# Hengle/AkariRender-1

Measured on AMD Instinct MI355X. Metric: Msamples/sec (whole node), 10M-tri scene 1080p 1024spp, 1/2/4/8 MI355X, higher is better.
Workload: dtype f32; 1 GPU; C3 synthetic triangle soup (SURVEY.md §8d); triangles=10000002, width=1920, height=1080, spp=1025, max_depth=5, tile=64, parallelism=tile-split x1, bvh_leaf=4, builder=sbvh, form=k_path, ordered_fetch=True

## Files before the change

akarirender-1_amd/csrc/kernels.hip:

```cpp
#include "akr_device.h"
#include "akr_math.h"
#include "kernels.h"
#include "leaf_layout.h"

namespace akr {

__device__ __forceinline__ uint32_t fbits(float f) { return __float_as_uint(f); }
__device__ __forceinline__ float bitsf(uint32_t u) { return __uint_as_float(u); }

template <bool TIGHT, bool FAST = false>
__device__ __forceinline__ float box_test(float lox, float hix, float loy, float hiy, float loz, float hiz, V3 o,
                                          V3 invd, float tmin, float tmax) {
    float t0x = (lox - o.x) * invd.x, t1x = (hix - o.x) * invd.x;
    float t0y = (loy - o.y) * invd.y, t1y = (hiy - o.y) * invd.y;
    float t0z = (loz - o.z) * invd.z, t1z = (hiz - o.z) * invd.z;
    float m0, m1, t;
    if (FAST) {
        m0 = fmaxf(fmaxf(fminf(t0x, t1x), fminf(t0y, t1y)), fminf(t0z, t1z));
        m1 = fminf(fminf(fmaxf(t0x, t1x), fmaxf(t0y, t1y)), fmaxf(t0z, t1z));
        t = fmaxf(tmin, m0);
    } else {
        m0 = rmax(rmax(rmin(t0x, t1x), rmin(t0y, t1y)), rmin(t0z, t1z));
        m1 = rmin(rmin(rmax(t0x, t1x), rmax(t0y, t1y)), rmax(t0z, t1z));
        t = rmax(tmin, m0);
// ... 225 lines not shown
            }
        }
    } else {
#pragma unroll
        for (int k = 0; k < 4; k++) {
            if ((rest >> pos[k]) & 1u) {
                const int e = sp + (int)__popc(rest >> (pos[k] + 1u));
                const unsigned long long v = (unsigned long long)ref[k] | ((unsigned long long)__float_as_uint(t[k]) << 32);
                if (e < kStackLds) lds_put(s_stack, e, tid, v);
                else ovf[(size_t)(e - kStackLds) * ovf_threads + gtid] = v;
            }
        }
    }
    sp += (int)__popc(rest);
    const uint32_t first = pm ^ rest;
    uint32_t c = AKR_CHILD_EMPTY;
#pragma unroll
    for (int k = 0; k < 4; k++) c = ((first >> pos[k]) & 1u) ? ref[k] : c;
    cur = c;
    return false;
}

template <bool TIGHT, bool ANY>
__device__ __forceinline__ int visit_wide(const float4 *wn, uint32_t &cur, V3 o, uint32_t dpos, V3 invd, float tmin, float tmax,
                                          float best, lds_u64 *s_stack, glb_u64 *ovf, uint32_t ovf_threads,
                                          uint32_t tid, uint32_t gtid, int &sp) {
    const char *wb = reinterpret_cast<const char *>(wn);
    const uint32_t off = cur << 6;
    const float4 h = *reinterpret_cast<const float4 *>(wb + off);
    const uint4 c = *reinterpret_cast<const uint4 *>(wb + off + 16);
    const uint4 qa = *reinterpret_cast<const uint4 *>(wb + off + 32);
    const uint4 qb = *reinterpret_cast<const uint4 *>(wb + off + 48);
    const uint32_t meta = __float_as_uint(h.w);
    const float sx = __uint_as_float((meta & 0xFFu) << 23);
    const float sy = __uint_as_float(((meta >> 8) & 0xFFu) << 23);
    const float sz = __uint_as_float(((meta >> 16) & 0xFFu) << 23);
    const float lim = ANY ? tmax : best;
    float t[4];
    bool hit[4];
    uint32_t ref[4] = {c.x, c.y, c.z, c.w};
#pragma unroll
    for (int k = 0; k < 4; k++) {
        const float lox = __builtin_fmaf(ubyte(qa.x, k), sx, h.x), hix = __builtin_fmaf(ubyte(qa.y, k), sx, h.x);
        const float loy = __builtin_fmaf(ubyte(qa.z, k), sy, h.y), hiy = __builtin_fmaf(ubyte(qa.w, k), sy, h.y);
        const float loz = __builtin_fmaf(ubyte(qb.x, k), sz, h.z), hiz = __builtin_fmaf(ubyte(qb.y, k), sz, h.z);
        t[k] = box_test<TIGHT, true>(lox, hix, loy, hiy, loz, hiz, o, invd, tmin, tmax);
        hit[k] = ref[k] != AKR_CHILD_EMPTY && !(t[k] < 0.0f || t[k] > lim);
    }
    const int tested = (c.x != AKR_CHILD_EMPTY) + (c.y != AKR_CHILD_EMPTY) + (c.z != AKR_CHILD_EMPTY) +
                       (c.w != AKR_CHILD_EMPTY);
    wide_order_push<ANY>(qb.z, qb.w, dpos, t, hit, ref, cur, lim, s_stack, ovf, ovf_threads, tid, gtid, sp);
    return tested;
}

struct WideNode {
    float4 h;
    uint4 c, qa, qb;
};
__device__ __forceinline__ WideNode wide_load(const float4 *wn, uint32_t cur) {
    const char *wb = reinterpret_cast<const char *>(wn);
    const uint32_t off = cur << 6;
    WideNode nd;
    nd.h = *reinterpret_cast<const float4 *>(wb + off);
    nd.c = *reinterpret_cast<const uint4 *>(wb + off + 16);
    nd.qa = *reinterpret_cast<const uint4 *>(wb + off + 32);
    nd.qb = *reinterpret_cast<const uint4 *>(wb + off + 48);
    return nd;
}

__device__ __forceinline__ float max3_raw(float a, float b, float c, float d) {
    float m, r;
    asm("v_max_f32 %0, %1, %2" : "=v"(m) : "v"(c), "v"(d));
    asm("v_max3_f32 %0, %1, %2, %3" : "=v"(r) : "v"(a), "v"(b), "v"(m));
    return r;
}
__device__ __forceinline__ float min3_raw(float a, float b, float c, float d) {
    float m, r;
    asm("v_min_f32 %0, %1, %2" : "=v"(m) : "v"(c), "v"(d));
    asm("v_min3_f32 %0, %1, %2, %3" : "=v"(r) : "v"(a), "v"(b), "v"(m));
    return r;
}

constexpr bool kTrimMinMax = true, kTrimPush = true;
template <bool ANY, bool NOPOP = false, bool FIT = false, bool TRIM = false>
__device__ __forceinline__ int visit_wide_lean_node(const WideNode &nd, uint32_t &cur, V3 o, uint32_t dpos, V3 invd,
                                                    float tmin, float tmaxp, float best, lds_u64 *s_stack, glb_u64 *ovf,
                                                    uint32_t ovf_threads, uint32_t tid, uint32_t gtid, int &sp,
                                                    bool *need_pop = nullptr, lds_u64 *dead = nullptr,
                                                    uint32_t *push_info = nullptr, uint32_t *entered = nullptr) {
    const float4 h = nd.h;
    const uint4 c = nd.c, qa = nd.qa, qb = nd.qb;
    const uint32_t meta = __float_as_uint(h.w);
    constexpr float kRel = 0x1p-21f;
    constexpr float kAbs = 0x1p-120f;
    const float scx = __uint_as_float((meta & 0xFFu) << 23) * invd.x;
    const float scy = __uint_as_float(((meta >> 8) & 0xFFu) << 23) * invd.y;
    const float scz = __uint_as_float(((meta >> 16) & 0xFFu) << 23) * invd.z;
    const float oqx = (h.x - o.x) * invd.x, oqy = (h.y - o.y) * invd.y, oqz = (h.z - o.z) * invd.z;
    const float ex = __builtin_fmaf(__builtin_fmaf(255.0f, fabsf(scx), fabsf(oqx)), kRel, kAbs);
    const float ey = __builtin_fmaf(__builtin_fmaf(255.0f, fabsf(scy), fabsf(oqy)), kRel, kAbs);
    const float ez = __builtin_fmaf(__builtin_fmaf(255.0f, fabsf(scz), fabsf(oqz)), kRel, kAbs);
    const float nox = oqx - ex, noy = oqy - ey, noz = oqz - ez;
    const float fox = oqx + ex, foy = oqy + ey, foz = oqz + ez;
    const bool px = invd.x > 0.0f, py = invd.y > 0.0f, pz = invd.z > 0.0f;
    const uint32_t qnx = px ? qa.x : qa.y, qfx = px ? qa.y : qa.x;
    const uint32_t qny = py ? qa.z : qa.w, qfy = py ? qa.w : qa.z;
    const uint32_t qnz = pz ? qb.x : qb.y, qfz = pz ? qb.y : qb.x;
    const float lim = ANY || TRIM ? tmaxp : fminf(best, tmaxp);
    float t[4];
    bool hit[4];
    uint32_t ref[4] = {c.x, c.y, c.z, c.w};
#pragma unroll
    for (int k = 0; k < 4; k++) {
        const float nx = __builtin_fmaf(ubyte(qnx, k), scx, nox), fx = __builtin_fmaf(ubyte(qfx, k), scx, fox);
        const float ny = __builtin_fmaf(ubyte(qny, k), scy, noy), fy = __builtin_fmaf(ubyte(qfy, k), scy, foy);
        const float nz = __builtin_fmaf(ubyte(qnz, k), scz, noz), fz = __builtin_fmaf(ubyte(qfz, k), scz, foz);
        constexpr bool RAW = TRIM && kTrimMinMax;
        const float tk = RAW ? max3_raw(nx, ny, nz, tmin) : fmaxf(fmaxf(nx, ny), fmaxf(nz, tmin));
        const float m1 = RAW ? min3_raw(fx, fy, fz, lim) : fminf(fminf(fx, fy), fminf(fz, lim));
        t[k] = tk;
        hit[k] = ref[k] != AKR_CHILD_EMPTY && tk <= m1;
    }
    const int tested = (c.x != AKR_CHILD_EMPTY) + (c.y != AKR_CHILD_EMPTY) + (c.z != AKR_CHILD_EMPTY) +
                       (c.w != AKR_CHILD_EMPTY);
    const bool np = wide_order_push<ANY, NOPOP, FIT, TRIM && kTrimPush>(qb.z, qb.w, dpos, t, hit, ref, cur, ANY ? tmaxp : best, s_stack, ovf,
                                                     ovf_threads, tid, gtid, sp, dead, push_info, entered);
    if (NOPOP) *need_pop = np;
    return tested;
}

template <bool ANY>
__device__ __forceinline__ int visit_wide_lean(const float4 *wn, uint32_t &cur, V3 o, uint32_t dpos, V3 invd, float tmin,
                                               float tmaxp, float best, lds_u64 *s_stack, glb_u64 *ovf,
                                               uint32_t ovf_threads, uint32_t tid, uint32_t gtid, int &sp) {
    const WideNode nd = wide_load(wn, cur);
    return visit_wide_lean_node<ANY>(nd, cur, o, dpos, invd, tmin, tmaxp, best, s_stack, ovf, ovf_threads, tid, gtid, sp);
}

__device__ __forceinline__ float float_below(float x) {
    const uint32_t b = __float_as_uint(x);
    if (x > 0.0f) return __uint_as_float(b - 1u);
    if (x == 0.0f) return -0x1p-149f;
    return __uint_as_float(b + 1u);
}

__device__ __forceinline__ bool lean_ok(V3 o, V3 invd, float tmin, float tmax) {
    const float mo = fmaxf(fmaxf(fabsf(o.x), fabsf(o.y)), fabsf(o.z));
    const float mi = fmaxf(fmaxf(fabsf(invd.x), fabsf(invd.y)), fabsf(invd.z));
    return fast_box_ok(o, invd, tmin, tmax) && tmin >= 0.0f && tmax > -INFINITY && mo <= 0x1p60f && mi <= 0x1p64f;
}

template <int MODE>
__device__ __forceinline__ void emit_result(const TraceArgs &a, uint32_t idx, float best, float bu, float bv,
                                            uint32_t bgid, bool occluded) {
    constexpr bool ANY = MODE != TRACE_CLOSEST;
    if (MODE == TRACE_SHADOW) {
        if (!occluded) {
            const float4 c = a.shadow_color[idx];
            const uint32_t slot = fbits(c.w);
            float4 l = a.L[slot];
            l.x += c.x;
            l.y += c.y;
            l.z += c.z;
            a.L[slot] = l;
        }
    } else if (a.abi_hits) {
// ... 1066 lines not shown
    unsigned long long tv_issue = 0, tv_wait = 0, tv_comp = 0, tl_issue = 0, tl_wait = 0, tl_comp = 0;
    unsigned long long lphases = 0, lholders = 0;
    unsigned long long pop_iters = 0, pop_rounds = 0, push_iters = 0, push_slow = 0, push_would_fit = 0;
    unsigned long long pop_lane_rounds = 0, pop_lanes = 0;
    bool deep_now = false;
    uint32_t *lines = nullptr;
    uint32_t span[3] = {0, 0, 0};
    const float4 *leaf_base = nullptr;
};

__device__ __forceinline__ void mark_lines(uint32_t *map, uint32_t lo, uint32_t hi, const void *region, const void *p,
                                           uint32_t bytes) {
    const uint64_t r0 = (uint64_t)region >> 7, a = (uint64_t)p;
    if (a < (uint64_t)region) return;
    for (uint64_t l = (a >> 7) - r0; l <= ((a + bytes - 1) >> 7) - r0; l++) {
        const uint64_t b = lo + l;
        if (b < hi) atomicOr(map + (b >> 5), 1u << (b & 31u));
    }
}

template <bool COUNT, bool OVF>
__device__ __forceinline__ void pop_bounded(bool need_pop, PathRay &r, const lds_u64 *s_stack, const glb_u64 *ovf,
                                            uint32_t ovf_threads, uint32_t tid, uint32_t gtid, uint32_t keep,
                                            uint32_t max_rounds, PathCount &c) {
    bool unserved = need_pop;
    uint32_t got = AKR_CHILD_POP;
    int sp = r.sp;
    uint32_t rounds = 0;
    while (true) {
        const bool has = unserved & (sp > 0);
        unsigned long long e;
        if constexpr (!OVF) {
            e = lds_get(s_stack, min(max(sp, 1), kStackLds) - 1, tid);
        } else {
            e = 0;
            if (has) {
                if (sp - 1 < kStackLds) e = lds_get(s_stack, sp - 1, tid);
                else e = ovf[(size_t)(sp - 1 - kStackLds) * ovf_threads + gtid];
            }
        }
        const bool ok = !(__uint_as_float((uint32_t)(e >> 32)) > r.best);
        const uint32_t got_entry = ok ? (uint32_t)e : got, got_none = unserved ? AKR_CHILD_EMPTY : got;
        got = has ? got_entry : got_none;
        sp -= has ? 1 : 0;
        if (COUNT) c.pop_lane_rounds += has ? 1 : 0;
        unserved = has & !ok;
        rounds++;
        if ((uint32_t)__popcll(__ballot(unserved)) < keep || rounds >= max_rounds) break;
    }
    if (COUNT) c.pop_rounds += rounds;
    r.sp = sp;
    if (need_pop) r.cur = got;
}

__device__ __forceinline__ unsigned long long mask_of(bool cmp) { return __builtin_amdgcn_ballot_w64(cmp); }
__device__ __forceinline__ bool in_mask(unsigned long long m) { return __builtin_amdgcn_inverse_ballot_w64(m); }
__device__ __forceinline__ uint32_t lane_count(unsigned long long m) {
    uint32_t n = (uint32_t)__popcll(m);
    asm("" : "+s"(n));
    return n;
}

__device__ __forceinline__ void pop_bounded_lds(unsigned long long need, PathRay &r, const lds_u64 *s_stack, uint32_t tid,
                                                uint32_t keep, uint32_t max_rounds) {
    unsigned long long unserved = need;
    uint32_t got = AKR_CHILD_POP;
    int sp = r.sp;
    uint32_t rounds = 0;
    while (true) {
        const unsigned long long has = unserved & mask_of(sp > 0);
        const unsigned long long e = lds_get(s_stack, min(max(sp, 1), kStackLds) - 1, tid);
        const unsigned long long cull = mask_of(__uint_as_float((uint32_t)(e >> 32)) > r.best);
        got = in_mask(unserved & ~has) ? AKR_CHILD_EMPTY : got;
        got = in_mask(has & ~cull) ? (uint32_t)e : got;
        sp -= in_mask(has) ? 1 : 0;
        unserved = has & cull;
        rounds++;
        if (lane_count(unserved) < (rounds < max_rounds ? keep : 65u)) break;
    }
    r.sp = sp;
    r.cur = in_mask(need) ? got : r.cur;
}

template <int EXIT>
__device__ __forceinline__ void path_traverse_masks(unsigned long long bm, PathRay &r, const float4 *wn, lds_u64 *s_stack,
                                                    glb_u64 *ovf, uint32_t ovf_threads, uint32_t tid, uint32_t gtid,
                                                    uint32_t pop_keep, uint32_t pop_rounds, lds_u64 *dead) {
    static_assert(EXIT >= 0 && EXIT < 64, "the exit test below counts a searching lane without a holder as 65");
    PathCount none;
    const float lim = fminf(r.best, r.tmaxp);
    while (true) {
        uint32_t pm = 1u;
        [[maybe_unused]] bool np;
        if (in_mask(bm & mask_of(is_internal(r.cur)))) {
            const WideNode nd = wide_load(wn, r.cur);
            visit_wide_lean_node<false, true, true, true>(nd, r.cur, r.o, r.dpos, r.invd, r.tmin, lim, r.best, s_stack,
                                                          ovf, ovf_threads, tid, gtid, r.sp, &np, dead, nullptr, &pm);
        }
        asm("" : "+v"(pm));
        unsigned long long need = mask_of(pm == 0);
        const unsigned long long no_leaf = mask_of(r.leaf == AKR_CHILD_EMPTY);
        const unsigned long long post = bm & ~need & no_leaf & mask_of(is_leaf(r.cur));
        r.leaf = in_mask(post) ? r.cur : r.leaf;
        need |= post | (bm & mask_of(r.cur == AKR_CHILD_POP));
        if (need != 0) {
            if (__builtin_expect((need & mask_of(r.sp > kStackLds)) == 0, 1))
                pop_bounded_lds(need, r, s_stack, tid, pop_keep, pop_rounds);
            else
                pop_bounded<false, true>(in_mask(need), r, s_stack, ovf, ovf_threads, tid, gtid, pop_keep, pop_rounds, none);
        }
        const unsigned long long free_now = bm & no_leaf & ~post;
        const unsigned long long searching = free_now & mask_of(r.cur != AKR_CHILD_EMPTY);
        const unsigned long long holders = bm & ~free_now;
        const uint32_t n = lane_count(searching);
        uint32_t left = holders != 0 ? n : n * 65u;
        asm("" : "+s"(left));
        if (left <= (uint32_t)EXIT) break;
    }
}

template <bool COUNT, int EXIT = kWhileExit, bool BOUND = false>
__device__ __forceinline__ void path_traverse(bool busy, int kind, PathRay &r, const float4 *wn, lds_u64 *s_stack,
                                              glb_u64 *ovf, uint32_t ovf_threads, uint32_t tid, uint32_t gtid,
                                              PathCount &c, uint32_t pop_keep = 1, uint32_t pop_rounds = 255,
                                              lds_u64 *dead = nullptr) {
    constexpr bool FIT = BOUND;
    while (true) {
        [[maybe_unused]] unsigned long long tc = 0;
        bool need_pop = false;
        if constexpr (COUNT) {
            c.strav++;
            c.sleaf += busy ? 1 : 0;
            c.iters++;
            const bool vis = busy && is_internal(r.cur);
            const unsigned long long ta = wall_clock64();
            const WideNode nd = wide_load(wn, vis ? r.cur : 0u);
            const unsigned long long tb = wall_clock64();
            asm volatile("s_waitcnt vmcnt(0)" ::: "memory");
            tc = wall_clock64();
            c.tv_issue += tb - ta;
            c.tv_wait += tc - tb;
            uint32_t pinfo = 0;
            if (vis) {
                const uint32_t node = r.cur;
                const int nt = visit_wide_lean_node<false, true, FIT>(nd, r.cur, r.o, r.dpos, r.invd, r.tmin, r.tmaxp,
                                                                      r.best, s_stack, ovf, ovf_threads, tid, gtid, r.sp,
                                                                      &need_pop, dead, &pinfo);
                c.box[kind] += nt;
                c.visit[kind]++;
                c.deep_now = c.deep_now || r.sp > kStackLds;
                if (c.lines)
                    mark_lines(c.lines, 0u, c.span[1], wn, reinterpret_cast<const char *>(wn) + ((size_t)node << 6), 64u);
            }
            if (__ballot(pinfo & 1u) != 0) {
                c.push_iters++;
                if (__ballot(pinfo & 2u) != 0) {
                    c.push_slow++;
                    c.push_would_fit += __ballot(pinfo & 4u) == 0 ? 1 : 0;
                }
            }
        } else if (busy && is_internal(r.cur)) {
            const WideNode nd = wide_load(wn, r.cur);
            visit_wide_lean_node<false, true, FIT>(nd, r.cur, r.o, r.dpos, r.invd, r.tmin, r.tmaxp, r.best, s_stack, ovf,
                                                   ovf_threads, tid, gtid, r.sp, &need_pop, dead);
        }
        if (busy && !need_pop && r.leaf == AKR_CHILD_EMPTY && is_leaf(r.cur)) {
            r.leaf = r.cur;
            need_pop = true;
        }
        if constexpr (BOUND) {
            need_pop = need_pop || (busy && r.cur == AKR_CHILD_POP);
            const unsigned long long want = __ballot(need_pop);
            if (want != 0) {
                if (COUNT) {
                    c.pop_iters++;
                    c.pop_lanes += need_pop ? 1 : 0;
                }
                if (__builtin_expect(__ballot(need_pop && r.sp > kStackLds) == 0, 1))
                    pop_bounded<COUNT, false>(need_pop, r, s_stack, ovf, ovf_threads, tid, gtid, pop_keep, pop_rounds, c);
                else
                    pop_bounded<COUNT, true>(need_pop, r, s_stack, ovf, ovf_threads, tid, gtid, pop_keep, pop_rounds, c);
            }
        } else {
            if (need_pop) r.cur = stack_pop(s_stack, ovf, ovf_threads, tid, gtid, r.sp, r.best);
        }
        const unsigned long long searching = __ballot(busy && r.leaf == AKR_CHILD_EMPTY && r.cur != AKR_CHILD_EMPTY);
        if constexpr (COUNT) {
            const bool stop = (uint32_t)__popcll(searching) <= (uint32_t)EXIT &&
                              (searching == 0 || __ballot(busy && r.leaf != AKR_CHILD_EMPTY) != 0);
            c.tv_comp += wall_clock64() - tc;
            if (stop) break;
        } else if ((uint32_t)__popcll(searching) <= (uint32_t)EXIT &&
                   (searching == 0 || __ballot(busy && r.leaf != AKR_CHILD_EMPTY) != 0)) {
            break;
        }
    }
}

template <bool COUNT>
// ... 9 lines not shown
    const uint32_t cnt = in ? fbits(l1.w) : 0u;
    const float4 *tp = lr + 2;
    for (uint32_t k = 0; k < cnt; k++) {
        if (COUNT && lane_prefix(__ballot(1)) == 0) c.stri += 64;
        const float4 ta = k == 0 ? pa0 : (k == 1 ? pa1 : tp[3 * k + 0]);
        const float4 tb = k == 0 ? pb0 : (k == 1 ? pb1 : tp[3 * k + 1]);
        const float4 tc = k == 0 ? pc0 : (k == 1 ? pc1 : tp[3 * k + 2]);
        if (COUNT) {
            c.tri[kind]++;
            if (c.lines && k >= 2) mark_lines(c.lines, c.span[1], c.span[2], c.leaf_base, tp + 3 * k, 48u);
        }
        float t, u, v;
        if (mt(r.o, r.d, r.tmin, r.tmax, ta, tb, tc, r.best, t, u, v)) {
            r.best = t;
            r.bu = u;
            r.bv = v;
            r.bgid = fbits(ta.w);
            if (kind) {
                hit_any = true;
                break;
            }
        }
    }
    r.leaf = AKR_CHILD_EMPTY;
    return hit_any;
}

template <bool COUNT>
__device__ __forceinline__ bool path_leaf(bool busy, int kind, PathRay &r, const float4 *wide_leaves, PathCount &c) {
    if constexpr (!COUNT) {
        bool hit_any = false;
        if (busy && r.leaf != AKR_CHILD_EMPTY) {
            const float4 *lr = wide_leaves + (r.leaf & kLeafOffsetMask);
            const float4 l0 = lr[0], l1 = lr[1];
            const float4 pa0 = lr[2], pb0 = lr[3], pc0 = lr[4];
            const float4 pa1 = lr[5], pb1 = lr[6], pc1 = lr[7];
            issue_together(pa0, pb0, pc0, pa1, pb1, pc1);
            const float tl = box_test<true, true>(l0.x, l0.w, l0.y, l1.x, l0.z, l1.y, r.o, r.invd, r.tmin, r.tmax);
            const bool in = !(tl < 0.0f || tl > r.best);
            const uint32_t cnt = in ? fbits(l1.w) : 0u;
            const float4 *tp = lr + 2;
            for (uint32_t k = 0; k < cnt; k++) {
                const float4 ta = k == 0 ? pa0 : (k == 1 ? pa1 : tp[3 * k + 0]);
                const float4 tb = k == 0 ? pb0 : (k == 1 ? pb1 : tp[3 * k + 1]);
                const float4 tc = k == 0 ? pc0 : (k == 1 ? pc1 : tp[3 * k + 2]);
                float t, u, v;
                if (mt(r.o, r.d, r.tmin, r.tmax, ta, tb, tc, r.best, t, u, v)) {
                    r.best = t;
                    r.bu = u;
                    r.bv = v;
                    r.bgid = fbits(ta.w);
                    if (kind) {
                        hit_any = true;
                        break;
                    }
                }
            }
            r.leaf = AKR_CHILD_EMPTY;
        }
        return hit_any;
    } else {
        bool hit_any = false;
        const unsigned long long ta = wall_clock64();
        const bool in_leaf = busy && r.leaf != AKR_CHILD_EMPTY;
        const uint32_t holders = (uint32_t)__popcll(__ballot(in_leaf));
        c.lphases += holders ? 1u : 0u;
        c.lholders += holders;
        const float4 *lr = wide_leaves + (in_leaf ? (r.leaf & kLeafOffsetMask) : 0u);
        const float4 l0 = lr[0], l1 = lr[1], pa0 = lr[2], pb0 = lr[3], pc0 = lr[4], pa1 = lr[5], pb1 = lr[6],
                     pc1 = lr[7];
        const unsigned long long tb = wall_clock64();
        asm volatile("s_waitcnt vmcnt(0)" ::: "memory");
        const unsigned long long tc = wall_clock64();
        if (in_leaf && c.lines) mark_lines(c.lines, c.span[1], c.span[2], wide_leaves, lr, 128u);
        if (in_leaf) hit_any = leaf_tests<true>(kind, r, lr, l0, l1, pa0, pb0, pc0, pa1, pb1, pc1, c);
        c.tl_issue += tb - ta;
        c.tl_wait += tc - tb;
        c.tl_comp += wall_clock64() - tc;
        return hit_any;
    }
}

__device__ __forceinline__ unsigned long long path_leaf_masks(unsigned long long bm, unsigned long long am, PathRay &r,
                                                              const float4 *wide_leaves) {
    const unsigned long long hold = bm & mask_of(r.leaf != AKR_CHILD_EMPTY);
    const unsigned long long one = hold & mask_of((r.leaf & kLeafOne) != 0);
    unsigned long long hm = 0;
    const bool several = hold != one;
    if (__builtin_expect(one != 0 && !several, 1)) {
        const float4 *lr = wide_leaves + (in_mask(one) ? (r.leaf & kLeafOffsetMask) : 0u);
        const float4 l0 = lr[0], l1 = lr[1];
        const float4 a = lr[2], b = lr[3], c = lr[4];
        const float tl = box_test<true, true>(l0.x, l0.w, l0.y, l1.x, l0.z, l1.y, r.o, r.invd, r.tmin, r.tmax);
        const unsigned long long out = mask_of(tl < 0.0f) | mask_of(tl > r.best);
        const V3 v0{a.x, a.y, a.z}, e1{b.x, b.y, b.z}, e2{c.x, c.y, c.z};
        const V3 h = cross(r.d, e2);
        const float det = dot(e1, h);
        const unsigned long long flat = mask_of(det > -1e-6f) & mask_of(det < 1e-6f);
        const float f = 1.0f / det;
        const V3 s = sub(r.o, v0);
        const float u = f * dot(s, h);
        const unsigned long long out_u = mask_of(u < 0.0f) | mask_of(u > 1.0f);
        const V3 q = cross(s, e1);
        const float v = f * dot(r.d, q);
        const unsigned long long out_v = mask_of(v < 0.0f) | mask_of(u + v > 1.0f);
        const float t = f * dot(e2, q);
        const unsigned long long near = mask_of(t > r.tmin) & mask_of(t < r.tmax) & mask_of(t < r.best);
        const unsigned long long hit = one & near & ~(out | flat | out_u | out_v);
        const bool won = in_mask(hit);
        r.best = won ? t : r.best;
        r.bu = won ? u : r.bu;
        r.bv = won ? v : r.bv;
        r.bgid = won ? fbits(a.w) : r.bgid;
        r.leaf = in_mask(one) ? AKR_CHILD_EMPTY : r.leaf;
        hm = hit & am;
    }
    if (__builtin_expect(several, 0)) {
        PathCount none{};
        hm |= mask_of(path_leaf<false>(in_mask(bm), in_mask(am) ? 1 : 0, r, wide_leaves, none));
    }
    return hm;
}

template <bool COUNT>
__device__ __forceinline__ bool path_begin(const TraceArgs &a, bool occl, float4 ra, float4 rb, PathRay &r,
                                           lds_u64 *s_stack, glb_u64 *ovf, uint32_t tid, uint32_t gtid, PathCount &c) {
    r.o = V3{ra.x, ra.y, ra.z};
    r.d = V3{rb.x, rb.y, rb.z};
    r.tmin = ra.w;
    r.tmax = rb.w;
    r.invd = V3{1.0f / r.d.x, 1.0f / r.d.y, 1.0f / r.d.z};
    r.dpos = (r.d.x > 0.0f ? 1u : 0u) | (r.d.y > 0.0f ? 2u : 0u) | (r.d.z > 0.0f ? 4u : 0u);
    if (occl && a.any_far_first) r.dpos ^= 7u;
    r.tmaxp = float_below(r.tmax);
    if (COUNT) c.rays[occl]++;
    if (!lean_ok(r.o, r.invd, r.tmin, r.tmax)) {
        bool hit;
        if (occl)
            trace_exact_core<true, true>(a, r.o, r.d, r.invd, r.tmin, r.tmax, s_stack, ovf, tid, gtid, r.best, r.bu,
                                         r.bv, r.bgid, hit);
        else
            trace_exact_core<false, true>(a, r.o, r.d, r.invd, r.tmin, r.tmax, s_stack, ovf, tid, gtid, r.best, r.bu,
                                          r.bv, r.bgid, hit);
        return false;
    }
    r.best = occl ? r.tmax : kInf;
    r.bu = r.bv = 0.0f;
    r.bgid = kNoHit;
    r.sp = 0;
    r.leaf = AKR_CHILD_EMPTY;
    if (COUNT) {
        c.box[occl]++;
        c.deep_now = false;
    }
    const float4 *nodesf = reinterpret_cast<const float4 *>(a.nodes);
    const float4 r0 = nodesf[0], r2 = nodesf[2];
    const float tr = box_test<true, true>(r0.x, r0.y, r0.z, r0.w, r2.x, r2.y, r.o, r.invd, r.tmin, r.tmax);
    r.cur = (a.wide_root == AKR_CHILD_EMPTY || tr < 0.0f || tr > r.best) ? AKR_CHILD_EMPTY : a.wide_root;
    return true;
}

__device__ __forceinline__ void path_park(uint32_t (*s_park)[kTraceBlock], uint32_t tid, const PathRay &r);
__device__ __forceinline__ void path_unpark(uint32_t (*s_park)[kTraceBlock], uint32_t tid, PathRay &r, bool far_first,
                                            bool occl);

struct PixelFetch {
    uint32_t shard, s_lo, s_hi;
    int shards_left;
    bool drained;
    uint32_t stride = 0;
};
__device__ __forceinline__ uint32_t gcd_u32(uint32_t x, uint32_t y) {
    while (y) {
        const uint32_t t = x % y;
        x = y;
        y = t;
    }
    return x;
}
__device__ __forceinline__ void fetch_pixels(PixelFetch &f, uint32_t n, uint32_t *work, uint32_t mode,
                                             const uint32_t *order, uint32_t prio, bool &need, bool &done,
                                             uint32_t &pix) {
    while (true) {
        const unsigned long long want = __ballot(need && !done);
        if (want == 0) break;
        if (f.drained) {
            if (need) done = true;
            break;
        }
        const uint32_t nw = (uint32_t)__popcll(want);
        const int leader = __ffsll((long long)want) - 1;
        uint32_t base = 0;
        if ((int)__lane_id() == leader) base = atomicAdd(work + f.shard * kWorkStride, nw);
        base = __builtin_amdgcn_readfirstlane(__shfl(base, leader));
        const uint32_t len = f.s_hi - f.s_lo;
        if (prio && base < len) {
            if ((uint64_t)base * 256u < (uint64_t)len * prio) __builtin_amdgcn_s_setprio(2);
            else __builtin_amdgcn_s_setprio(0);
        }
        if (need && !done) {
            const uint32_t my = base + lane_prefix(want);
            if (base < len && my < len) {
// ... 61 lines not shown
        atomicAdd(&q.pop_iters, c.pop_iters);
        atomicAdd(&q.pop_rounds, c.pop_rounds);
        atomicAdd(&q.push_iters, c.push_iters);
        atomicAdd(&q.push_slow, c.push_slow);
        atomicAdd(&q.push_would_fit, c.push_would_fit);
    }
    const unsigned long long plr = wave_sum(c.pop_lane_rounds), pln = wave_sum(c.pop_lanes);
    if (__lane_id() == 0 && pa.prof) {
        atomicAdd(&pa.prof->pop_lane_rounds, plr);
        atomicAdd(&pa.prof->pop_lanes, pln);
    }
    const int slot_of[2] = {TRACE_CLOSEST, TRACE_SHADOW};
    for (int m = 0; m < 2; m++) {
        const unsigned long long rr = wave_sum(c.rays[m]), b = wave_sum(c.box[m]), t = wave_sum(c.tri[m]),
                                 v = wave_sum(c.visit[m]), dp = wave_sum(c.deep[m]), lf = wave_sum(c.leaf[m]);
        if (__lane_id() == 0) {
            TraceCounters &tc = a.counters[slot_of[m]];
            atomicAdd(&tc.rays, rr);
            atomicAdd(&tc.box, b);
            atomicAdd(&tc.tri, t);
            atomicAdd(&tc.visits, v);
            atomicAdd(&tc.deep, dp);
            atomicAdd(&tc.leaves, lf);
        }
    }
    const unsigned long long st = wave_sum(c.strav), sl = wave_sum(c.sleaf), sr = wave_sum(c.stri);
    if (__lane_id() == 0) {
        atomicAdd(&a.counters[TRACE_CLOSEST].slots_trav, st);
        atomicAdd(&a.counters[TRACE_CLOSEST].slots_leaf, sl);
        atomicAdd(&a.counters[TRACE_CLOSEST].slots_tri, sr);
    }
}

template <bool COUNT>
__device__ __forceinline__ uint32_t probe_flags(const PathArgs &pa) {
    if (!COUNT) return AKR_PROBE_SEED;
    uint32_t f = AKR_PROBE_SEED | AKR_PROBE_RAYS;
    if (pa.probe_clock) f |= 4u | (uint32_t)((wall_clock64() >> 4) << 8);
    return f;
}

constexpr int kParkSlots = 8;

template <bool COUNT, bool TAB, bool ONE, bool SIMPLE, bool ENV = false>
__device__ __forceinline__ void path_plain(const PathArgs &pa, const EnvDev *env = nullptr) {
    if (pa.gate && *pa.gate != pa.gate_want) return;
    const TraceArgs &a = pa.t;
    __shared__ unsigned long long s_stack_mem[kStackLdsU64];
    __shared__ uint32_t s_park[kParkSlots][kTraceBlock];
    __shared__ uint4 s_tab[TAB ? kTabBytes / 16 : 1];
    lds_u64 *s_stack = (lds_u64 *)s_stack_mem;
    glb_u64 *stack_ovf = (glb_u64 *)a.stack_ovf;
    const uint32_t tid = threadIdx.x;
    const uint32_t gtid = blockIdx.x * kTraceBlock + tid;
    const uint32_t n = pa.n_pix;
    const int nb = pa.max_depth == 0 ? 1 : pa.max_depth;
    const bool ff = a.any_far_first != 0;
    const auto tab = PathTab<TAB>::make(pa.sc, s_tab);
    static_assert(kParkSlots >= 1 && kTraceBlock % 64 == 0, "the push's scratch words lie in a wave's park row 0");
    lds_u64 *dead = (lds_u64 *)&s_park[0][0] + (tid >> 1);
    PathCount c;
    if (COUNT) {
        c.lines = pa.lines;
        c.span[1] = pa.lines_span[1];
        c.span[2] = pa.lines_span[2];
        c.leaf_base = a.wide_leaves;
    }
    PixelFetch f{blockIdx.x % kWorkShards, 0, 0, (int)kWorkShards, n == 0};
    f.s_lo = shard_begin(n, f.shard);
    f.s_hi = shard_begin(n, f.shard + 1);

    uint32_t pix = 0, left = 0, seed = 0, pxr = 0;
    int depth = 0;
    V3 beta{1.0f, 1.0f, 1.0f}, Lr{0.0f, 0.0f, 0.0f}, scol{0.0f, 0.0f, 0.0f};
    float4 film = {0.0f, 0.0f, 0.0f, 0.0f};
    float4 pe0 = {}, pe1 = {};
    enum : uint32_t { F_BUSY = 1u, F_DONE = 2u, F_FIN = 4u, F_NEED = 8u, F_ANY = 16u, F_PEND = 32u };
    uint32_t fl = F_NEED;
    uint32_t pc_closest = 0, pc_shadow = 0;
    PathRay r{};
    r.best = kInf;
    r.bgid = kNoHit;
    r.cur = r.leaf = AKR_CHILD_EMPTY;
    unsigned long long p_outer = 0, p_procs = 0, p_tp = 0, p_tt = 0, p_tl = 0, p_lanes = 0, p_t0 = 0, p_t = 0, p_tsh = 0;
    unsigned long long p_tpark = 0, p_tnext = 0, p_tbegin = 0, p_tload = 0;
    if (COUNT) p_t0 = wall_clock64();

    while (true) {
        const unsigned long long waiting = mask_of((fl & (F_BUSY | F_DONE)) == 0);
        const uint32_t nwait = (uint32_t)__popcll(waiting);
        const uint32_t nbusy = (uint32_t)__popcll(mask_of((fl & F_BUSY) != 0));
        if (nwait == 0 && nbusy == 0) break;
        if (COUNT) {
            p_outer++;
            p_t = wall_clock64();
        }
        if (nwait > 0 && 64u * nwait >= pa.min_wait * (nwait + nbusy)) {
            if (COUNT) {
                p_procs++;
                p_lanes += nwait;
            }
            bool busy = (fl & F_BUSY) != 0, done = (fl & F_DONE) != 0, fin = (fl & F_FIN) != 0;
            bool need_pixel = (fl & F_NEED) != 0, any = (fl & F_ANY) != 0, pend = (fl & F_PEND) != 0;
            path_park(s_park, tid, r);
            __builtin_amdgcn_fence(__ATOMIC_RELEASE, "workgroup");
            asm volatile("" ::: "memory");
            bool fresh = false, next_any = false, sample_end = false, start = false;
            float4 ra = {}, rb = {};
            unsigned long long p_ts = 0;
            unsigned long long tl_phase = 0;
            if (COUNT) {
                p_ts = wall_clock64();
                p_tpark += p_ts - p_t;
            }
            if (!busy && !done && fin) {
                fin = false;
                const uint32_t hgid = r.bgid;
                [[maybe_unused]] const EnvDev *envp = env;
                if constexpr (ENV) {
                    unsigned long long eb = (unsigned long long)env;
                    asm volatile("" : "+s"(eb));
                    envp = (const EnvDev *)(const AKR_GLOBAL EnvDev *)eb;
                }
                if (any) {
                    if (hgid == kNoHit) {
                        Lr.x += scol.x;
                        Lr.y += scol.y;
                        Lr.z += scol.z;
                    }
                    if (pend) {
                        ra = pe0;
                        rb = pe1;
                        fresh = true;
                        pend = false;
                    } else {
                        sample_end = true;
                    }
                } else if (hgid == kNoHit) {
                    if constexpr (ENV) {
                        if (depth == 0) {
                            const V3 d{bitsf(s_park[3][tid]), bitsf(s_park[4][tid]), bitsf(s_park[5][tid])};
                            int ti, tj;
                            float len;
                            env_encode(envp->n, env_to_map(*envp, d), ti, tj, len);
                            const V3 e = mul(beta, env_lookup(*envp, ti, tj));
                            Lr.x += e.x;
                            Lr.y += e.y;
                            Lr.z += e.z;
                        }
                    }
                    sample_end = true;
                } else {
                    const V3 wo{-bitsf(s_park[3][tid]), -bitsf(s_park[4][tid]), -bitsf(s_park[5][tid])};
                    Bounce bo;
                    if (COUNT && pa.lines)
                        mark_lines(pa.lines, pa.lines_span[2], pa.lines_span[3], pa.sc.tri, pa.sc.tri + hgid,
                                   (uint32_t)sizeof(ShadeTri));
                    shade_hit_path<SIMPLE, ENV>(pa.sc, tab, hgid, r.bu, r.bv, wo, beta, seed, depth,
                                                pa.max_depth, depth == nb - 1, bo, COUNT ? &tl_phase : nullptr, envp);
                    if (bo.emit) {
                        Lr.x += bo.e.x;
                        Lr.y += bo.e.y;
                        Lr.z += bo.e.z;
                    }
                    if (bo.ext) {
                        beta = bo.nb;
                        depth++;
                    }
                    if (bo.sh) {
                        ra = bo.s0;
                        rb = bo.s1;
                        scol = bo.col;
                        next_any = true;
                        fresh = true;
                        pend = bo.ext;
                        pe0 = bo.e0;
                        pe1 = bo.e1;
                    } else if (bo.ext) {
                        ra = bo.e0;
                        rb = bo.e1;
                        fresh = true;
                    } else {
                        sample_end = true;
                    }
                }
            }
            if (COUNT) {
                const unsigned long long t = wall_clock64();
                p_tsh += t - p_ts;
                p_ts = t;
                p_tload += wave_max(tl_phase);
            }
            if (sample_end) {
                splat_one(film, make_float4(Lr.x, Lr.y, Lr.z, 0.0f), pa.ray_clamp);
                if (--left == 0) {
                    pa.film[pix] = film;
                    if (pa.state_out) pa.state_out[pix] = seed;
                    if (pa.probe)
                        pa.probe[pix] = make_uint4(seed, COUNT ? pc_closest : 0u, COUNT ? pc_shadow : 0u,
                                                   probe_flags<COUNT>(pa));
                    need_pixel = true;
                } else {
                    start = true;
                }
            }
            const bool asked = need_pixel && !done;
            fetch_pixels(f, n, pa.work, pa.order ? pa.order_mode : FETCH_LINEAR, pa.order, pa.prio, need_pixel, done, pix);
            if (asked && !need_pixel) {
                const uint32_t px = pa.pixel[pix];
                pxr = px;
                left = pa.spp;
                if (pa.state_in) {
                    seed = pa.state_in[pix];
                    film = pa.film[pix];
                } else {
                    seed = (uint32_t)((int)(px & 0xFFFFu) + (int)(px >> 16) * pa.cam.width);
                    film = make_float4(0.0f, 0.0f, 0.0f, 0.0f);
                }
                start = true;
                if (COUNT) pc_closest = pc_shadow = 0;
            }
            if (start) {
                Lr = V3{0.0f, 0.0f, 0.0f};
                beta = V3{1.0f, 1.0f, 1.0f};
                depth = 0;
                const uint32_t px = pxr;
                camera_ray(pa.cam, (int)(px & 0xFFFFu), (int)(px >> 16), seed, ra, rb);
                fresh = true;
            }
            asm volatile("" ::: "memory");
            if (COUNT) {
                const unsigned long long t = wall_clock64();
                p_tnext += t - p_ts;
                p_ts = t;
            }
            path_unpark(s_park, tid, r, ff, any);
            if (fresh) {
                any = next_any;
                if (COUNT) {
                    pc_closest += any ? 0u : 1u;
                    pc_shadow += any ? 1u : 0u;
                }
                busy = path_begin<COUNT>(a, any, ra, rb, r, s_stack, stack_ovf, tid, gtid, c);
                fin = !busy;
            }
            fl = (busy ? F_BUSY : 0u) | (done ? F_DONE : 0u) | (fin ? F_FIN : 0u) | (need_pixel ? F_NEED : 0u) |
                 (any ? F_ANY : 0u) | (pend ? F_PEND : 0u);
            asm("" : "+v"(fl));
            if (COUNT) p_tbegin += wall_clock64() - p_ts;
        }
        if (COUNT) {
            const unsigned long long t = wall_clock64();
            p_tp += t - p_t;
            p_t = t;
        }
        const unsigned long long bm = mask_of((fl & F_BUSY) != 0);
        if (bm == 0) continue;
        const bool busy = in_mask(bm);
        [[maybe_unused]] const int kd = (fl & F_ANY) != 0 ? 1 : 0;
        if constexpr (COUNT)
            path_traverse<COUNT, kWhileExitPath, true>(busy, kd, r, a.wide_nodes, s_stack, stack_ovf, a.ovf_threads, tid,
                                                       gtid, c, pa.pop_keep, pa.pop_rounds, dead);
        else
            path_traverse_masks<kWhileExitPath>(bm, r, a.wide_nodes, s_stack, stack_ovf, a.ovf_threads, tid, gtid,
                                                pa.pop_keep, pa.pop_rounds, dead);
        if (COUNT) {
            const unsigned long long t = wall_clock64();
            p_tt += t - p_t;
            p_t = t;
        }
        bool ended;
        if constexpr (COUNT || !ONE) {
            const bool hit_any = path_leaf<COUNT>(busy, kd, r, a.wide_leaves, c);
            ended = busy && (hit_any || r.cur == AKR_CHILD_EMPTY);
        } else {
            const unsigned long long hm = path_leaf_masks(bm, mask_of((fl & F_ANY) != 0), r, a.wide_leaves);
            ended = in_mask(bm & (hm | mask_of(r.cur == AKR_CHILD_EMPTY)));
        }
        fl = ended ? (fl ^ (F_BUSY | F_FIN)) : fl;
        if (COUNT && ended) c.deep[kd] += c.deep_now ? 1 : 0;
        if (COUNT) p_tl += wall_clock64() - p_t;
    }
    if (COUNT) {
        path_count_flush(pa, c, p_outer, p_procs, p_tp, p_tt, p_tl, p_t0, p_lanes, p_tsh);
        if (__lane_id() == 0 && pa.prof) {
            atomicAdd(&pa.prof->tp_park, p_tpark);
            atomicAdd(&pa.prof->tp_next, p_tnext);
            atomicAdd(&pa.prof->tp_begin, p_tbegin);
            atomicAdd(&pa.prof->tp_load, p_tload);
        }
    }
}

template <bool COUNT, bool TAB>
__global__ __launch_bounds__(kTraceBlock) __attribute__((amdgpu_waves_per_eu(AKR_PATH_WAVES))) void k_path(PathArgs pa) {
    path_plain<COUNT, TAB, true, !COUNT>(pa);
}
template <bool TAB, bool SIMPLE>
__global__ __launch_bounds__(kTraceBlock) __attribute__((amdgpu_waves_per_eu(AKR_PATH_WAVES))) void k_path_general(PathArgs pa) {
    path_plain<false, TAB, false, SIMPLE>(pa);
}
template <bool COUNT, bool TAB>
__global__ __launch_bounds__(kTraceBlock) __attribute__((amdgpu_waves_per_eu(AKR_PATH_WAVES))) void k_path_env(PathEnvArgs ea) {
    path_plain<COUNT, TAB, true, !COUNT, true>(ea.p, (const EnvDev *)ea.env);
}
template <bool TAB, bool SIMPLE>
__global__ __launch_bounds__(kTraceBlock) __attribute__((amdgpu_waves_per_eu(AKR_PATH_WAVES))) void k_path_env_general(PathEnvArgs ea) {
    path_plain<false, TAB, false, SIMPLE, true>(ea.p, (const EnvDev *)ea.env);
}

__device__ __forceinline__ void path_park(uint32_t (*s_park)[kTraceBlock], uint32_t tid, const PathRay &r) {
    const float pv[8] = {r.o.x, r.o.y, r.o.z, r.d.x, r.d.y, r.d.z, r.tmin, r.tmax};
#pragma unroll
    for (int k = 0; k < 8; k++) s_park[k][tid] = fbits(pv[k]);
}
__device__ __forceinline__ void path_unpark(uint32_t (*s_park)[kTraceBlock], uint32_t tid, PathRay &r, bool far_first,
                                            bool occl) {
    r.o = V3{bitsf(s_park[0][tid]), bitsf(s_park[1][tid]), bitsf(s_park[2][tid])};
    r.d = V3{bitsf(s_park[3][tid]), bitsf(s_park[4][tid]), bitsf(s_park[5][tid])};
    r.tmin = bitsf(s_park[6][tid]);
    r.tmax = bitsf(s_park[7][tid]);
    r.invd = V3{1.0f / r.d.x, 1.0f / r.d.y, 1.0f / r.d.z};
    r.dpos = (r.d.x > 0.0f ? 1u : 0u) | (r.d.y > 0.0f ? 2u : 0u) | (r.d.z > 0.0f ? 4u : 0u);
    if (occl && far_first) r.dpos ^= 7u;
    r.tmaxp = float_below(r.tmax);
    r.leaf = AKR_CHILD_EMPTY;
}

__device__ __forceinline__ int nth_set_bit(unsigned long long m, uint32_t r) {
    int base = 0;
#pragma unroll
    for (int s = 32; s > 0; s >>= 1) {
        const unsigned long long low = m & ((1ull << s) - 1ull);
        const uint32_t c = (uint32_t)__popcll(low);
        if (r >= c) {
            r -= c;
            m >>= s;
            base += s;
        } else {
            m = low;
        }
    }
    return base;
}

constexpr uint32_t kDeferSlots = 8;
enum : uint32_t { RAY_NONE = 0, RAY_OWN = 1, RAY_OWN_SHADOW = 2, RAY_FOREIGN = 3 };

struct DeferState {
    uint32_t w = 0;
    static constexpr uint32_t KIND = 0, RP = 2, LAST = 3, OPEN = 4, NSH = 6, DEPTH = 14, FTAG = 18, PEND = 30, RUN = 31;
    __device__ __forceinline__ uint32_t get(uint32_t off, uint32_t bits) const { return (w >> off) & ((1u << bits) - 1u); }
    __device__ __forceinline__ void set(uint32_t off, uint32_t bits, uint32_t v) {
        const uint32_t m = ((1u << bits) - 1u) << off;
        w = (w & ~m) | ((v << off) & m);
    }
    __device__ __forceinline__ uint32_t kind() const { return get(KIND, 2); }
    __device__ __forceinline__ uint32_t rp() const { return get(RP, 1); }
    __device__ __forceinline__ uint32_t last() const { return get(LAST, 1); }
// ... 1298 lines not shown
```

Baseline: 621.1 Msamples/s.

## Prefetch next wide BVH node across loop iterations and trim leaf loads

Issues the load of the next internal wide node at the end of each traversal iteration, after leaf processing and after ray begin, and carries it in registers so the next visit starts with data already in flight. Inline asm barriers keep the node registers live and grouped with the leaf loads so the memory latency overlaps the leaf test. Leaf fetches shrink to float2/float3 loads where only some components are used. The node limit switches to float_below(tmax). This adds around 16 VGPRs of live state per lane, which can lower occupancy, and the change spans several call sites whose consistency must hold.

```diff
diff --git a/akarirender-1_amd/csrc/kernels.hip b/akarirender-1_amd/csrc/kernels.hip
--- a/akarirender-1_amd/csrc/kernels.hip
+++ b/akarirender-1_amd/csrc/kernels.hip
@@ -331,6 +331,26 @@
 }
 
 constexpr bool kTrimMinMax = true, kTrimPush = true;
+constexpr bool kNodeAhead = true;
+__device__ __forceinline__ void node_together(const WideNode &nd) {
+    asm volatile("" ::"v"(nd.h.x), "v"(nd.h.y), "v"(nd.h.z), "v"(nd.h.w), "v"(nd.c.x), "v"(nd.c.y), "v"(nd.c.z),
+                 "v"(nd.c.w), "v"(nd.qa.x), "v"(nd.qa.y), "v"(nd.qa.z), "v"(nd.qa.w), "v"(nd.qb.x), "v"(nd.qb.y),
+                 "v"(nd.qb.z), "v"(nd.qb.w));
+}
+__device__ __forceinline__ void node_forget(WideNode &nd) {
+    asm volatile("" : "=v"(nd.h.x), "=v"(nd.h.y), "=v"(nd.h.z), "=v"(nd.h.w), "=v"(nd.c.x), "=v"(nd.c.y), "=v"(nd.c.z),
+                 "=v"(nd.c.w), "=v"(nd.qa.x), "=v"(nd.qa.y), "=v"(nd.qa.z), "=v"(nd.qa.w), "=v"(nd.qb.x),
+                 "=v"(nd.qb.y), "=v"(nd.qb.z), "=v"(nd.qb.w));
+}
+__device__ __forceinline__ void node_here(WideNode &nd) {
+    asm volatile("" : "+v"(nd.h.x), "+v"(nd.h.y), "+v"(nd.h.z), "+v"(nd.h.w), "+v"(nd.c.x), "+v"(nd.c.z), "+v"(nd.qa.x),
+                 "+v"(nd.qa.y), "+v"(nd.qa.z), "+v"(nd.qa.w), "+v"(nd.qb.x), "+v"(nd.qb.y), "+v"(nd.qb.z),
+                 "+v"(nd.qb.w));
+    uint32_t c1, c3;
+    asm volatile("v_mov_b32 %0, %2\n\tv_mov_b32 %1, %3" : "=&v"(c1), "=&v"(c3) : "v"(nd.c.y), "v"(nd.c.w));
+    nd.c.y = c1;
+    nd.c.w = c3;
+}
 template <bool ANY, bool NOPOP = false, bool FIT = false, bool TRIM = false>
 __device__ __forceinline__ int visit_wide_lean_node(const WideNode &nd, uint32_t &cur, V3 o, uint32_t dpos, V3 invd,
                                                     float tmin, float tmaxp, float best, lds_u64 *s_stack, glb_u64 *ovf,
@@ -1563,19 +1583,24 @@
     r.cur = in_mask(need) ? got : r.cur;
 }
 
-template <int EXIT>
+__device__ __forceinline__ void node_ahead(unsigned long long vm, WideNode &nd, const float4 *wn, uint32_t cur) {
+    node_forget(nd);
+    if (in_mask(vm)) nd = wide_load(wn, cur);
+}
+template <int EXIT, bool AHEAD>
 __device__ __forceinline__ void path_traverse_masks(unsigned long long bm, PathRay &r, const float4 *wn, lds_u64 *s_stack,
                                                     glb_u64 *ovf, uint32_t ovf_threads, uint32_t tid, uint32_t gtid,
-                                                    uint32_t pop_keep, uint32_t pop_rounds, lds_u64 *dead) {
+                                                    uint32_t pop_keep, uint32_t pop_rounds, lds_u64 *dead, WideNode &nd) {
     static_assert(EXIT >= 0 && EXIT < 64, "the exit test below counts a searching lane without a holder as 65");
     PathCount none;
-    const float lim = fminf(r.best, r.tmaxp);
+    const float lim = fminf(r.best, AHEAD ? float_below(r.tmax) : r.tmaxp);
     while (true) {
         uint32_t pm = 1u;
         [[maybe_unused]] bool np;
         if (in_mask(bm & mask_of(is_internal(r.cur)))) {
-            const WideNode nd = wide_load(wn, r.cur);
-            visit_wide_lean_node<false, true, true, true>(nd, r.cur, r.o, r.dpos, r.invd, r.tmin, lim, r.best, s_stack,
+            WideNode now = AHEAD ? nd : wide_load(wn, r.cur);
+            if constexpr (AHEAD) node_here(now);
+            visit_wide_lean_node<false, true, true, true>(now, r.cur, r.o, r.dpos, r.invd, r.tmin, lim, r.best, s_stack,
                                                           ovf, ovf_threads, tid, gtid, r.sp, &np, dead, nullptr, &pm);
         }
         asm("" : "+v"(pm));
@@ -1596,6 +1621,7 @@
         const uint32_t n = lane_count(searching);
         uint32_t left = holders != 0 ? n : n * 65u;
         asm("" : "+s"(left));
+        if constexpr (AHEAD) node_ahead(bm & mask_of(is_internal(r.cur)), nd, wn, r.cur);
         if (left <= (uint32_t)EXIT) break;
     }
 }
@@ -1771,15 +1797,25 @@
 }
 
 __device__ __forceinline__ unsigned long long path_leaf_masks(unsigned long long bm, unsigned long long am, PathRay &r,
-                                                              const float4 *wide_leaves) {
+                                                              const float4 *wide_leaves, WideNode &nd, const float4 *wn) {
     const unsigned long long hold = bm & mask_of(r.leaf != AKR_CHILD_EMPTY);
     const unsigned long long one = hold & mask_of((r.leaf & kLeafOne) != 0);
     unsigned long long hm = 0;
     const bool several = hold != one;
     if (__builtin_expect(one != 0 && !several, 1)) {
         const float4 *lr = wide_leaves + (in_mask(one) ? (r.leaf & kLeafOffsetMask) : 0u);
-        const float4 l0 = lr[0], l1 = lr[1];
-        const float4 a = lr[2], b = lr[3], c = lr[4];
+        const float4 l0 = lr[0];
+        const float2 l1h = *reinterpret_cast<const float2 *>(lr + 1);
+        const float4 l1 = kNodeAhead ? make_float4(l1h.x, l1h.y, 0.0f, 0.0f) : lr[1];
+        const float4 a = lr[2];
+        const float3 b3 = *reinterpret_cast<const float3 *>(lr + 3), c3 = *reinterpret_cast<const float3 *>(lr + 4);
+        const float4 b = kNodeAhead ? make_float4(b3.x, b3.y, b3.z, 0.0f) : lr[3];
+        const float4 c = kNodeAhead ? make_float4(c3.x, c3.y, c3.z, 0.0f) : lr[4];
+        if constexpr (kNodeAhead) {
+            asm volatile("" ::"v"(l0.x), "v"(l0.y), "v"(l0.z), "v"(l0.w), "v"(l1h.x), "v"(l1h.y), "v"(a.x), "v"(a.y), "v"(a.z),
+                         "v"(a.w), "v"(b3.x), "v"(b3.y), "v"(b3.z), "v"(c3.x), "v"(c3.y), "v"(c3.z));
+            node_together(nd);
+        }
         const float tl = box_test<true, true>(l0.x, l0.w, l0.y, l1.x, l0.z, l1.y, r.o, r.invd, r.tmin, r.tmax);
         const unsigned long long out = mask_of(tl < 0.0f) | mask_of(tl > r.best);
         const V3 v0{a.x, a.y, a.z}, e1{b.x, b.y, b.z}, e2{c.x, c.y, c.z};
@@ -1807,6 +1843,7 @@
     if (__builtin_expect(several, 0)) {
         PathCount none{};
         hm |= mask_of(path_leaf<false>(in_mask(bm), in_mask(am) ? 1 : 0, r, wide_leaves, none));
+        if constexpr (kNodeAhead) node_ahead(bm & mask_of(is_internal(r.cur)), nd, wn, r.cur);
     }
     return hm;
 }
@@ -2034,6 +2071,8 @@
     r.best = kInf;
     r.bgid = kNoHit;
     r.cur = r.leaf = AKR_CHILD_EMPTY;
+    constexpr bool AHEAD = kNodeAhead && !COUNT && ONE;
+    WideNode nd;
     unsigned long long p_outer = 0, p_procs = 0, p_tp = 0, p_tt = 0, p_tl = 0, p_lanes = 0, p_t0 = 0, p_t = 0, p_tsh = 0;
     unsigned long long p_tpark = 0, p_tnext = 0, p_tbegin = 0, p_tload = 0;
     if (COUNT) p_t0 = wall_clock64();
@@ -2199,6 +2238,8 @@
             fl = (busy ? F_BUSY : 0u) | (done ? F_DONE : 0u) | (fin ? F_FIN : 0u) | (need_pixel ? F_NEED : 0u) |
                  (any ? F_ANY : 0u) | (pend ? F_PEND : 0u);
             asm("" : "+v"(fl));
+            if constexpr (AHEAD)
+                node_ahead(mask_of((fl & F_BUSY) != 0) & mask_of(is_internal(r.cur)), nd, a.wide_nodes, r.cur);
             if (COUNT) p_tbegin += wall_clock64() - p_ts;
         }
         if (COUNT) {
@@ -2214,8 +2255,8 @@
             path_traverse<COUNT, kWhileExitPath, true>(busy, kd, r, a.wide_nodes, s_stack, stack_ovf, a.ovf_threads, tid,
                                                        gtid, c, pa.pop_keep, pa.pop_rounds, dead);
         else
-            path_traverse_masks<kWhileExitPath>(bm, r, a.wide_nodes, s_stack, stack_ovf, a.ovf_threads, tid, gtid,
-                                                pa.pop_keep, pa.pop_rounds, dead);
+            path_traverse_masks<kWhileExitPath, AHEAD>(bm, r, a.wide_nodes, s_stack, stack_ovf, a.ovf_threads, tid, gtid,
+                                                pa.pop_keep, pa.pop_rounds, dead, nd);
         if (COUNT) {
             const unsigned long long t = wall_clock64();
             p_tt += t - p_t;
@@ -2226,7 +2267,7 @@
             const bool hit_any = path_leaf<COUNT>(busy, kd, r, a.wide_leaves, c);
             ended = busy && (hit_any || r.cur == AKR_CHILD_EMPTY);
         } else {
-            const unsigned long long hm = path_leaf_masks(bm, mask_of((fl & F_ANY) != 0), r, a.wide_leaves);
+            const unsigned long long hm = path_leaf_masks(bm, mask_of((fl & F_ANY) != 0), r, a.wide_leaves, nd, a.wide_nodes);
             ended = in_mask(bm & (hm | mask_of(r.cur == AKR_CHILD_EMPTY)));
         }
         fl = ended ? (fl ^ (F_BUSY | F_FIN)) : fl;
```

Result: no change. 619.0 Msamples/s (-0.3%).
